# WangYuTum/odometry

Measured on AMD Instinct MI355X. Metric: tracked frames/sec (1241x376, 4-level pyramid), higher is better.
Workload: dtype f32

## Files before the change

### odometry_amd/csrc/kernels.hip.h

```cpp
#pragma once
#include <hip/hip_runtime.h>
#include "odo_math.h"

#ifndef ODO_PHASE_STAMPS
#define ODO_PHASE_STAMPS 0
#endif
#if ODO_PHASE_STAMPS
#define ODO_DBG(a) ((a).dbg)
#else
#define ODO_DBG(a) ((unsigned long long*)nullptr)
#endif

#ifndef ODO_KERNEL
#define ODO_KERNEL __global__
#define ODO_KERNEL_T __global__
#endif
#ifdef ODO_LM_CHAIN_TU
#define ODO_DEVICE_VAR static __device__
#else
#define ODO_DEVICE_VAR __device__
#endif

namespace odo {

// ... 1154 lines not shown
    if (lv) {
      while (!h.active && h.status == 0 && !h.finished) {
        const int next = (h.level < 0) ? n_levels - 1 : h.level - 1;
        if (next < stop_level) { h.finished = 1; break; }
        h.stop_reason = 0;
        h.level = next;
        h.iter = 0;
        h.err_last = 1e+10f;
        h.lambda = lambda0;
        h.inc = h.cur;
        h.max_iters = lv[next].max_iters;
        h.active = (h.status == 0 && h.max_iters > 0) ? 1 : 0;
#pragma unroll
        for (int c = 0; c < 4; c++) {
#pragma unroll
          for (int r = 0; r < 3; r++) Tn[c * 4 + r] = h.Tc[c * 3 + r];
          Tn[c * 4 + 3] = (c == 3) ? 1.0f : 0.0f;
        }
        new_T = true;
      }
      if (h.status != 0) h.finished = 1;
    }
    if (t == 0) {
      if (new_T) {
#pragma unroll
        for (int i = 0; i < 16; i++) s_sh.T[i] = Tn[i];
      }
      s_sh.level = h.level; s_sh.active = h.active; s_sh.status = h.status; s_sh.finished = h.finished;
    }
  }
  __syncthreads();
}

constexpr int kUpdThreads = 1024;
#define ODO_STAMP(i) do { if (STAMP && threadIdx.x == 0) stamps[i] = __builtin_readcyclecounter(); } while (0)
template <bool STAMP>
__device__ __forceinline__ void lm_update_body(LmState* __restrict__ st, const double* __restrict__ partials,
                                               int nblk, int expect_level, float precision, int max_iters,
                                               LmTraceRow* __restrict__ trace, float* __restrict__ cost_stat,
                                               int* __restrict__ host_prog, int seq,
                                               unsigned long long* __restrict__ stamps) {
  ODO_STAMP(0);
  if (!(st->active != 0 && st->level == expect_level)) {
    if (host_prog && threadIdx.x == 0) __hip_atomic_store(host_prog, seq, __ATOMIC_RELAXED, __HIP_MEMORY_SCOPE_SYSTEM);
    return;
  }
  __shared__ double sh[32][32];
  __shared__ double acc_sh[32];
  __shared__ LmState s_sh;
  const int t = threadIdx.x;
  const int q = t & 31, seg = t >> 5;
  double v = 0.0;
  if (q < ODO_NACC) {
    double v0 = 0.0, v1 = 0.0, v2 = 0.0, v3 = 0.0;
    int b = seg;
    for (; b + 96 < nblk; b += 128) {
      v0 += partials[(size_t)b * ODO_NACC + q];
      v1 += partials[(size_t)(b + 32) * ODO_NACC + q];
      v2 += partials[(size_t)(b + 64) * ODO_NACC + q];
      v3 += partials[(size_t)(b + 96) * ODO_NACC + q];
    }
    for (; b < nblk; b += 32) v0 += partials[(size_t)b * ODO_NACC + q];
    v = (v0 + v1) + (v2 + v3);
  }
  ODO_STAMP(1);
  sh[seg][q] = v;
// ... 232 lines not shown
  for (int rd = 0; rd < kCoarseRounds; rd++) my_cnt[rd] = __popcll(__ballot(rd < nr && valid[rd]));
  float sigma = 5.0f;
  int n_total = 0;
  for (int pass = 0; pass < kTdistMaxPasses; pass++) {
#pragma unroll
    for (int rd = 0; rd < kCoarseRounds; rd++) {
      const double ws = wave_sum64((rd < nr && valid[rd]) ? (double)tdist_term(e2[rd], sigma * sigma) : 0.0);
      if (lane == 0) { part[pass & 1][rd * kW + wv] = ws; if (pass == 0) cnt[rd * kW + wv] = my_cnt[rd]; }
    }
    __syncthreads();
    if (pass == 0) {
      int tot = 0;
#pragma unroll
      for (int i = 0; i < kCoarseChunks; i++) tot += cnt[i];
      n_total = tot;
    }
    double G = 0.0;
    if (lane < kCoarseChunks / 4) {
      const double* pv = &part[pass & 1][(lane >> 1) * kW + 4 * (lane & 1)];
      G = ((pv[0] + pv[1]) + pv[2]) + pv[3];
    }
    const double total = wave_sum64(G);
    const float nxt = (n_total > 0) ? tdist_next_sigma(total, n_total) : sigma;
    const bool done = (n_total == 0) || tdist_converged(nxt, sigma);
    sigma = nxt;
    if (done) break;
  }
  return sigma;
}
#if ODO_PHASE_STAMPS
ODO_DEVICE_VAR unsigned long long g_lm_diag[24];
#endif
constexpr unsigned long long kArmWaitTicks = 200000000ull;
template <bool kFull, bool kArmed = false>
__device__ __forceinline__ void lm_coarse_body(const StepArgs& a, const StepLaunch& q, int min_level, const unsigned* __restrict__ lv_src) {
#if ODO_PHASE_STAMPS
  const unsigned long long w_entry = (unsigned long long)wall_clock64();
#endif
  if (!kArmed && lm_chain_skip(a)) return;
  __builtin_amdgcn_s_setprio(3);
  lm_span_begin(q.span);
  __shared__ LmState s_sh;
  extern __shared__ __attribute__((aligned(16))) double red_sh[];
  __shared__ double acc_sh[32];
  __shared__ StepLevel lv_sh[ODO_MAX_LEVELS_K];
  __shared__ unsigned long long sm_sh[4];
  unsigned long long arm_g0 = 0;
  if (kArmed && threadIdx.x < 17) arm_g0 = __hip_atomic_load(a.arm + threadIdx.x, __ATOMIC_RELAXED, __HIP_MEMORY_SCOPE_SYSTEM);
  lm_copy_levels(lv_sh, lv_src);
  if (threadIdx.x == 0) {
#pragma unroll
    for (int i = 0; i < 4; i++) sm_sh[i] = 0;
  }
  __shared__ __attribute__((aligned(16))) float arm_pose_sh[16];
  __shared__ __attribute__((aligned(16))) int arm_verdict_sh4[4];
  if (kArmed) {
    if (threadIdx.x < 64) {
      const int lane = (int)threadIdx.x;
      unsigned long long g = arm_g0;
      bool got = __all(lane >= 17 || (int)(g >> 32) == a.token);
      const unsigned long long t0 = (unsigned long long)wall_clock64();
      for (int spin = 0; !got; spin++) {
        if (lane < 17) g = __hip_atomic_load(a.arm + lane, __ATOMIC_RELAXED, __HIP_MEMORY_SCOPE_SYSTEM);
        got = __all(lane >= 17 || (int)(g >> 32) == a.token);
        if (!got && (spin & 15) == 15 && (unsigned long long)wall_clock64() - t0 > (a.fine_wait ? (unsigned long long)a.fine_wait : kArmWaitTicks)) break;
      }
      if (lane < 16) arm_pose_sh[lane] = __uint_as_float((unsigned)g);
      if (lane == 16) arm_verdict_sh4[0] = got ? (int)(unsigned)g : 3;
    }
    __syncthreads();
    if (arm_verdict_sh4[0] == 3) {
      if (threadIdx.x < 64) {
        if (threadIdx.x < (int)(sizeof(LmState) / sizeof(int))) ((int*)&s_sh)[threadIdx.x] = 0;
        if (threadIdx.x == 0) { s_sh.status = -2; s_sh.active = 0; s_sh.finished = 1; }
      }
      __syncthreads();
      lm_fused_publish(s_sh, q.st_out, a.host_prog, q.seq, a.token, a.cost_stat, a.out, a.done_flag, a.final_state);
      return;
    }
    if (arm_verdict_sh4[0] != 1) return;
  } else {
    __syncthreads();
  }
#if ODO_PHASE_STAMPS
  const unsigned long long w_p1 = (unsigned long long)wall_clock64();
#endif
  lm_fused_prologue(q.st_in, q.part_in, lv_sh, a.n_levels, a.lambda0, a.precision, s_sh, red_sh, acc_sh, (kFull ? a.trace : (LmTraceRow*)nullptr), a.cost_stat, true,
                    kArmed ? arm_pose_sh : (q.first_of_solve ? a.init : nullptr), a.stop_level, (!kArmed && a.chain_in_token) ? a.chain_pose : nullptr);
#if ODO_PHASE_STAMPS
  const unsigned long long w_p2 = (unsigned long long)wall_clock64();
#endif
  LmHot hot;
  lm_hot_load(hot, s_sh);
  if (ODO_DBG(a) && threadIdx.x == 0 && q.seq < 56) ODO_DBG(a)[16 + 2 * q.seq] = wall_clock64();
  unsigned long long c_eval = 0, c_red = 0, c_sm = 0, c_it = 0, c_last = ODO_DBG(a) ? __builtin_readcyclecounter() : 0;
  const unsigned long long c_begin = c_last, w_begin = ODO_DBG(a) ? (unsigned long long)wall_clock64() : 0;
  auto lap = [&](unsigned long long& sum) {
    if (ODO_DBG(a)) { const unsigned long long now = __builtin_readcyclecounter(); sum += now - c_last; c_last = now; }
  };
  static_assert(kCoarseBlock == 2 * kLmBlock, "two 256-point virtual blocks per round");
  constexpr int kS = 8;
  constexpr int kVbMax = (kCoarseMaxPoints + kLmBlock - 1) / kLmBlock;
  __shared__ double part_sh[kVbMax][32];
  __shared__ double sc_part[2][kCoarseChunks];
  __shared__ int sc_cnt[kCoarseChunks];
  const int tl = threadIdx.x & (kLmBlock - 1), half = threadIdx.x >> 8;
  float* rows_sh = (float*)red_sh + half * (kRowFloats * RowBuf<kLmBlock>::W);
  const int my_q = tl / kS, my_s = tl % kS;
  int rowA = 0, rowB = 0;
  if (my_q < ODO_NACC) rows_of_quantity(my_q, &rowA, &rowB);
  PointK cpt[kCoarseRounds];
  bool cpt_ok[kCoarseRounds] = {false, false};
  int cpt_level = -1;
  for (int guard = 0; guard < 4096; guard++) {
    const bool run = (s_sh.active != 0 && s_sh.status == 0 && s_sh.level >= min_level);
    if (!run) break;
    c_it++;
    const StepLevel& L = lv_sh[s_sh.level];
    const float* I2u = lm_uniform_ptr(L.I2);
    float T[16];
#pragma unroll
    for (int i = 0; i < 16; i++) T[i] = s_sh.T[i];
    const int nvb = L.nblk;
    if (s_sh.level != cpt_level) {
      cpt_level = s_sh.level;
#pragma unroll
      for (int rd = 0; rd < kCoarseRounds; rd++) {
        const int vb = 2 * rd + half, idx = vb * kLmBlock + tl;
        cpt_ok[rd] = vb < nvb && idx < L.n;
        if (cpt_ok[rd]) cpt[rd] = load_point(L.pl, idx);
      }
    }
    float td_r[kCoarseRounds] = {0.0f, 0.0f}, td_J[kCoarseRounds][6] = {{0.0f, 0.0f, 0.0f, 0.0f, 0.0f, 0.0f}, {0.0f, 0.0f, 0.0f, 0.0f, 0.0f, 0.0f}};
    bool td_valid[kCoarseRounds] = {false, false};
    float td_scale_sqr = 1.0f;
    if ((kFull && a.robust == 2)) {
      float e2[kCoarseRounds];
#pragma unroll
      for (int rd = 0; rd < kCoarseRounds; rd++) {
        if (cpt_ok[rd]) td_valid[rd] = point_residual_g<kFull>(cpt[rd], T, L.k, I2u, L.rows, L.cols, &td_r[rd], td_J[rd]);
        e2[rd] = td_r[rd] * td_r[rd];
      }
      const float sg = coarse_tdist_sigma(sc_part, sc_cnt, e2, td_valid, (nvb + 1) / 2);
      td_scale_sqr = sg * sg;
    }
#pragma unroll
    for (int vb0 = 0; vb0 < 2 * kCoarseRounds; vb0 += 2) {
      if (vb0 >= nvb) break;
      const int vb = vb0 + half;
      float r = 0.0f, w = 0.0f, J[6] = {0.0f, 0.0f, 0.0f, 0.0f, 0.0f, 0.0f};
      bool valid = false;
      if ((kFull && a.robust == 2)) {
        r = td_r[vb0 / 2]; valid = td_valid[vb0 / 2];
#pragma unroll
        for (int i = 0; i < 6; i++) J[i] = td_J[vb0 / 2][i];
// ... 8 lines not shown
      rows_store_z(rows_sh, RowBuf<kLmBlock>::W, tl, J, w, r, valid);
      __syncthreads();
      if (vb0 == 0) lap(c_eval);
      double accq = 0.0;
      if (vb < nvb) {
        if (my_q < ODO_NACC) accq = rows_accumulate<kLmBlock, kS>(rows_sh, rowA, rowB, my_s, accq);
        accq = rows_butterfly8(accq);
      }
      if (nvb == 1) {
        if (half == 0 && my_q < ODO_NACC && my_s == 0) {
          double v = 0.0;
          v += accq;
          double acc = 0.0;
          acc += v;
#pragma unroll
          for (int g = 1; g < 8; g++) acc += 0.0;
          acc_sh[my_q] = acc;
        }
      } else if (vb < nvb && my_q < ODO_NACC && my_s == 0) {
        part_sh[vb][my_q] = accq;
      }
    }
    __syncthreads();
    if (nvb > 1) {
      const int fq = threadIdx.x & 31, fseg = threadIdx.x >> 5;
      double* fold_sh = red_sh;
      if (fseg < 8) {
        double v = 0.0;
        if (fq < ODO_NACC)
          for (int b = fseg; b < nvb; b += 8) v += part_sh[b][fq];
        fold_sh[fseg * 32 + fq] = v;
      }
      __syncthreads();
      if (threadIdx.x < ODO_NACC) {
        double acc = 0.0;
#pragma unroll
        for (int g = 0; g < 8; g++) acc += fold_sh[g * 32 + threadIdx.x];
        acc_sh[threadIdx.x] = acc;
      }
    }
    lap(c_red);
    lm_state_machine_hot(hot, lv_sh, a.n_levels, a.lambda0, a.precision, s_sh, acc_sh, (kFull ? a.trace : (LmTraceRow*)nullptr), a.cost_stat, true,
                         ODO_DBG(a) ? sm_sh : nullptr, a.stop_level);
    lap(c_sm);
  }
#if ODO_PHASE_STAMPS
  const unsigned long long w_loop_end = (unsigned long long)wall_clock64();
#endif
  if (threadIdx.x == 0) lm_hot_store(hot, s_sh);
  lm_fused_publish(s_sh, q.st_out, a.host_prog, q.seq, a.token, a.cost_stat, a.out, a.done_flag, a.final_state, chain_out_of(a));
#if ODO_PHASE_STAMPS
  if (ODO_DBG(a) && threadIdx.x == 0) {
    const unsigned long long now = (unsigned long long)wall_clock64();
    g_lm_diag[4] += w_begin - w_entry; g_lm_diag[5] += w_loop_end - w_begin; g_lm_diag[6] += now - w_loop_end;
    g_lm_diag[16] += w_p1 - w_entry; g_lm_diag[17] += w_p2 - w_p1; g_lm_diag[18] += w_begin - w_p2;
    if (g_lm_diag[1] && w_entry > g_lm_diag[1] && w_entry - g_lm_diag[1] < 100000ull) { g_lm_diag[7] += w_entry - g_lm_diag[1]; g_lm_diag[3] += w_entry - g_lm_diag[2]; g_lm_diag[14] += 1; }
    g_lm_diag[0] = now; g_lm_diag[8] += 1;
  }
#endif
  if (ODO_DBG(a) && threadIdx.x == 0) {
    if (q.seq < 56) ODO_DBG(a)[16 + 2 * q.seq + 1] = wall_clock64();
    ODO_DBG(a)[0] += c_eval; ODO_DBG(a)[1] += c_red; ODO_DBG(a)[2] += c_sm; ODO_DBG(a)[3] += c_it;
    ODO_DBG(a)[4] += __builtin_readcyclecounter() - c_begin; ODO_DBG(a)[5] += 1;
    ODO_DBG(a)[6] += (unsigned long long)wall_clock64() - w_begin;
#pragma unroll
    for (int i = 0; i < 4; i++) ODO_DBG(a)[8 + i] += sm_sh[i];
  }
  lm_span_end(q.span);
}

#ifdef ODO_LM_CHAIN_TU
static __global__ void __launch_bounds__(kCoarseBlock) lm_coarse_kernel(StepArgs a, int min_level) {
  const StepLaunch q = {a.st_in, a.st_out, a.part_in, a.part_out, a.seq, a.first_of_solve, a.span};
  lm_coarse_body<false>(a, q, min_level, lm_kernarg_words());
}
static __global__ void __launch_bounds__(kCoarseBlock) lm_coarse_armed_kernel(StepArgs a, int min_level) {
  const StepLaunch q = {a.st_in, a.st_out, a.part_in, a.part_out, a.seq, a.first_of_solve, a.span};
  lm_coarse_body<false, true>(a, q, min_level, lm_kernarg_words());
}
static __global__ void __launch_bounds__(kCoarseBlock) lm_coarse_full_kernel(StepArgs a, int min_level) {
  const StepLaunch q = {a.st_in, a.st_out, a.part_in, a.part_out, a.seq, a.first_of_solve, a.span};
  lm_coarse_body<true>(a, q, min_level, lm_kernarg_words());
}
#endif
template <bool kFull>
__device__ __forceinline__ void lm_coarse_batch_entry(const StepArgs* __restrict__ table, int seq, int first_of_solve, unsigned long long* span) {
  const StepArgs& a = table[blockIdx.y];
  const StepLaunch q = {a.st2[seq & 1], a.st2[(seq + 1) & 1], a.part2[seq & 1], a.part2[(seq + 1) & 1], seq, first_of_solve, span};
  lm_coarse_body<kFull>(a, q, a.min_level, (const unsigned*)&table[blockIdx.y]);
}
ODO_KERNEL void __launch_bounds__(kCoarseBlock) lm_coarse_kernel_batch(const StepArgs* __restrict__ table, int seq, int first_of_solve,
                                                                       unsigned long long* span) {
  lm_coarse_batch_entry<false>(table, seq, first_of_solve, span);
}
ODO_KERNEL void __launch_bounds__(kCoarseBlock) lm_coarse_full_kernel_batch(const StepArgs* __restrict__ table, int seq, int first_of_solve,
                                                                            unsigned long long* span) {
  lm_coarse_batch_entry<true>(table, seq, first_of_solve, span);
}

constexpr int kFineGran = 2 * ODO_NACC;
constexpr int kFineRowsMax = 160;
constexpr int kFineChunk = 8;
constexpr unsigned kFineWaitTicks = 400000u;
struct FineDeadline {
  unsigned long long t0, c0;
  unsigned limit;
  static __device__ __forceinline__ FineDeadline begin(unsigned limit_ticks) {
    return FineDeadline{(unsigned long long)wall_clock64(), (unsigned long long)__builtin_readcyclecounter(), limit_ticks};
  }
  __device__ __forceinline__ bool expired(int spin) const {
    if ((spin & 31) != 31) return false;
// ... 157 lines not shown
    }
    FineG2 g = {0, 0, 0, 0};
    unsigned long long gc = 0;
    bool all = false;
    FineDeadline dl = {0ull, 0ull, wait_limit};
    __builtin_amdgcn_s_setprio(0);
    for (int spin = 0; !all; spin++) {
      if (spin == 1) dl = FineDeadline::begin(wait_limit);
      if (spin > 0) { if (dl.expired(spin)) break; __builtin_amdgcn_s_sleep(1); }
      bool mine = true;
      if (lane < nvb) {
        g = *(const volatile FineG2Global*)(sums + 2 * lane);
        if (pass == 0) gc = __hip_atomic_load(cnts + lane, __ATOMIC_RELAXED, __HIP_MEMORY_SCOPE_AGENT);
        mine = (g.x == tag) && (g.z == tag) && (pass != 0 || (unsigned)gc == tag);
      }
      all = __all(mine);
    }
    __builtin_amdgcn_s_setprio(3);
    if (!all) { if (lane == 0) *bail = 1; break; }
    double part = 0.0, cnt = 0.0;
    if (lane < nvb) {
      part = __longlong_as_double((long long)(((unsigned long long)g.y << 32) | (unsigned long long)g.w));
      if (pass == 0) cnt = (double)(unsigned)(gc >> 32);
    }
    const double total = wave_sum64(part);
    if (pass == 0) n_total = (int)wave_sum64(cnt);
    const float nxt = (n_total > 0) ? tdist_next_sigma(total, n_total) : sigma;
    const bool done = (n_total == 0) || tdist_converged(nxt, sigma);
    sigma = nxt;
    if (done) break;
  }
  return sigma;
}
template <bool kTdist, bool kTrace>
__device__ __forceinline__ void lm_fine_body(const StepArgs& a, const StepLaunch& q, int K, int w, unsigned long long* __restrict__ xbuf,
                                             int fault, int lo_level, const unsigned* __restrict__ lv_src) {
#if ODO_PHASE_STAMPS
  const unsigned long long w_entry = (unsigned long long)wall_clock64();
#endif
  __builtin_amdgcn_s_setprio(3);
  const int t = threadIdx.x, tl = t & (kLmBlock - 1), half = t >> 8;
  const bool publisher = (w == 0);
  if (publisher && t == 0 && q.span) atomicMin(q.span, (unsigned long long)wall_clock64());
  __shared__ LmState s_sh;
  __shared__ double fold_sh[8 * 32];
  __shared__ double acc_sh[32];
  __shared__ StepLevel lv_sh[ODO_MAX_LEVELS_K];
  __shared__ float rows_sh2[2][kRowFloats * RowBuf<kLmBlock>::W];
  __shared__ int bail_sh, local_sh;
  __shared__ unsigned long long sm_sh[4];
  float* rows_sh = rows_sh2[half];
  const unsigned tag_base = a.fine_epoch << 8;
  unsigned long long* place = xbuf + 2 * kFineRowsMax * kFineGran;
  const unsigned wait_limit = a.fine_wait ? a.fine_wait : kFineWaitTicks;
  lm_copy_levels(lv_sh, lv_src);
  if (t == 0) {
    bail_sh = 0;
    local_sh = 0;
#pragma unroll
    for (int i = 0; i < 4; i++) sm_sh[i] = 0;
    __hip_atomic_store(place + w, ((unsigned long long)(unsigned)fine_xcc_id() << 32) | tag_base, __ATOMIC_RELAXED, __HIP_MEMORY_SCOPE_AGENT);
  }
  __syncthreads();
  lm_fused_prologue(q.st_in, q.part_in, lv_sh, a.n_levels, a.lambda0, a.precision, s_sh, fold_sh, acc_sh, (kTrace ? a.trace : (LmTraceRow*)nullptr), a.cost_stat,
                    publisher, q.first_of_solve ? a.init : nullptr, a.stop_level, a.chain_in_token ? a.chain_pose : nullptr);
  LmHot hot;
  lm_hot_load(hot, s_sh);
  if (t < 64) {
    bool same = true, got = false;
    if (t < K) {
      unsigned long long pw = 0;
      const FineDeadline dl = FineDeadline::begin(wait_limit);
      for (int spin = 0; !got; spin++) {
        pw = __hip_atomic_load(place + t, __ATOMIC_RELAXED, __HIP_MEMORY_SCOPE_AGENT);
        got = ((unsigned)pw == tag_base);
        if (!got && dl.expired(spin)) break;
      }
      same = got && ((int)(pw >> 32) == fine_xcc_id());
    } else {
      got = true;
    }
    const bool all_got = __all(got), all_same = __all(same);
    if (t == 0) { local_sh = (all_got && all_same) ? 1 : 0; if (!all_got) bail_sh = 1; }
  }
  __syncthreads();
  const bool local = local_sh != 0;
  constexpr int kS = 8;
  const int my_q = tl / kS, my_s = tl % kS;
  int rowA = 0, rowB = 0;
  if (my_q < ODO_NACC) rows_of_quantity(my_q, &rowA, &rowB);
  const int fq = t & 31, fseg = t >> 5;
  PointK pt;
  bool pt_ok = false;
  int pt_level = -1;
  unsigned long long c_eval = 0, c_xchg = 0, c_sm = 0, c_it = 0, c_last = ODO_DBG(a) ? __builtin_readcyclecounter() : 0;
#if ODO_PHASE_STAMPS
  unsigned long long c_first = 0, n_first = 0;
#endif
  const unsigned long long c_begin = c_last, w_begin = ODO_DBG(a) ? (unsigned long long)wall_clock64() : 0;
  auto lap = [&](unsigned long long& sum) {
    if (ODO_DBG(a)) { const unsigned long long now = __builtin_readcyclecounter(); sum += now - c_last; c_last = now; }
  };
  for (int ev = 0; ev < 4096; ev++) {
    const bool run = (s_sh.active != 0 && s_sh.status == 0 && !s_sh.finished && !bail_sh && s_sh.level >= lo_level);
    if (!run) break;
    c_it++;
    const StepLevel& L = lv_sh[s_sh.level];
    const float* I2u = lm_uniform_ptr(L.I2);
    const int nblk = L.nblk;
    const unsigned tag = tag_base + 1u + (unsigned)(ev % 255);
    unsigned long long* buf = xbuf + (size_t)(ev & 1) * kFineRowsMax * kFineGran;
    float T[16];
#pragma unroll
    for (int i = 0; i < 16; i++) T[i] = s_sh.T[i];
#if ODO_PHASE_STAMPS
    const bool first_of_level = (s_sh.level != pt_level);
#endif
    const bool resident = (nblk <= 2 * K) && (L.n <= nblk * kLmBlock);
    if (resident) {
      const int vb = w + half * K;
      if (s_sh.level != pt_level) {
        pt_level = s_sh.level;
        const int idx = vb * kLmBlock + tl;
        pt_ok = vb < nblk && idx < L.n;
        if (pt_ok) pt = load_point(L.pl, idx);
      }
      float r = 0.0f, wgt = 0.0f, J[6] = {0.0f, 0.0f, 0.0f, 0.0f, 0.0f, 0.0f};
      bool valid = false;
      if (pt_ok && point_residual_g<kTdist || kTrace>(pt, T, L.k, I2u, L.rows, L.cols, &r, J)) {
        wgt = robust_weight(r, (kTdist || kTrace) ? a.robust : (a.robust == 1 ? 1 : 0), a.huber_delta, 1.0f);
        valid = true;
      }
      if (kTdist && w < nblk) {
        __shared__ double td_ws_sh[2][8];
        __shared__ int td_cnt_sh[8];
        const float sg = fine_tdist_sigma(xbuf + kFineScaleOff, vb * 4 + (tl >> 6), 4 * nblk,
                                          ((a.fine_epoch & 0xfffu) << 20) | (((unsigned)ev & 0x3ffu) << 10), r * r, valid, local, wait_limit, &bail_sh,
                                          td_ws_sh, td_cnt_sh);
        if (valid) wgt = robust_weight(r, 2, a.huber_delta, sg * sg);
      }
      rows_store_z(rows_sh, RowBuf<kLmBlock>::W, tl, J, wgt, r, valid);
      __syncthreads();
      if (bail_sh) break;
      if (vb < nblk) {
        double accq = 0.0;
        if (my_q < ODO_NACC) accq = rows_accumulate<kLmBlock, kS>(rows_sh, rowA, rowB, my_s, accq);
        accq = rows_butterfly8(accq);
// ... 32 lines not shown
    double v = 0.0;
    __builtin_amdgcn_s_setprio(0);
    if (fq < ODO_NACC && fseg < 8) {
      for (int b0 = fseg; b0 < nblk; b0 += 8 * kFineChunk) {
        FineG2 g2[kFineChunk];
        bool all = false;
        FineDeadline dl = {0ull, 0ull, wait_limit};
        for (int spin = 0; !all; spin++) {
          if (spin == 1) dl = FineDeadline::begin(wait_limit);
          if (spin > 0) { if (dl.expired(spin)) break; __builtin_amdgcn_s_sleep(1); }
          all = true;
#pragma unroll
          for (int u = 0; u < kFineChunk; u++) {
            const int b = b0 + 8 * u;
            if (b < nblk) g2[u] = *(const volatile FineG2Global*)(buf + (size_t)b * kFineGran + 2 * fq);
          }
#pragma unroll
          for (int u = 0; u < kFineChunk; u++) {
            const int b = b0 + 8 * u;
            if (b < nblk) all = all && (g2[u].x == tag) && (g2[u].z == tag);
          }
        }
        if (!all) bail_sh = 1;
#pragma unroll
        for (int u = 0; u < kFineChunk; u++) {
          const int b = b0 + 8 * u;
          if (b < nblk) v += __longlong_as_double((long long)(((unsigned long long)g2[u].y << 32) | (unsigned long long)g2[u].w));
        }
      }
    }
    __builtin_amdgcn_s_setprio(3);
    if (fseg < 8) fold_sh[fseg * 32 + fq] = v;
    __syncthreads();
    if (t < ODO_NACC) {
      double acc = 0.0;
#pragma unroll
      for (int g = 0; g < 8; g++) acc += fold_sh[g * 32 + t];
      acc_sh[t] = acc;
    }
    lap(c_xchg);
    if (bail_sh) break;
    lm_state_machine_hot(hot, lv_sh, a.n_levels, a.lambda0, a.precision, s_sh, acc_sh, (kTrace ? a.trace : (LmTraceRow*)nullptr), a.cost_stat, publisher,
                         (ODO_DBG(a) && publisher) ? sm_sh : nullptr, a.stop_level);
    lap(c_sm);
  }
#if ODO_PHASE_STAMPS
  const unsigned long long w_loop_end = (unsigned long long)wall_clock64();
#endif
  if (t == 0) lm_hot_store(hot, s_sh);
  if (bail_sh && t == 0) { s_sh.status = -2; s_sh.active = 0; s_sh.finished = 1; }
  __syncthreads();
  if (publisher) {
    lm_fused_publish(s_sh, q.st_out, a.host_prog, q.seq, a.token, a.cost_stat, a.out, a.done_flag, a.final_state, chain_out_of(a));
#if ODO_PHASE_STAMPS
    const unsigned long long w_published = (unsigned long long)wall_clock64();
#endif
    if (ODO_DBG(a) && t == 0) { ODO_DBG(a)[128] += c_eval; ODO_DBG(a)[129] += c_xchg; ODO_DBG(a)[130] += c_sm; ODO_DBG(a)[131] += c_it; ODO_DBG(a)[132] += 1; ODO_DBG(a)[133] += local ? 1 : 0;
      ODO_DBG(a)[134] += __builtin_readcyclecounter() - c_begin; ODO_DBG(a)[135] += (unsigned long long)wall_clock64() - w_begin;
#pragma unroll
      for (int i = 0; i < 4; i++) ODO_DBG(a)[136 + i] += sm_sh[i]; }
    if (t == 0 && q.span) atomicMax(q.span + 1, (unsigned long long)wall_clock64());
#if ODO_PHASE_STAMPS
    if (ODO_DBG(a) && t == 0) {
      const unsigned long long now = w_published;
      g_lm_diag[2] = w_loop_end;
      g_lm_diag[19] += c_first; g_lm_diag[20] += n_first;
      g_lm_diag[9] += w_begin - w_entry; g_lm_diag[10] += w_loop_end - w_begin; g_lm_diag[11] += now - w_loop_end;
      if (g_lm_diag[0] && w_entry > g_lm_diag[0] && w_entry - g_lm_diag[0] < 100000ull) { g_lm_diag[12] += w_entry - g_lm_diag[0]; g_lm_diag[15] += 1; }
      g_lm_diag[1] = now; g_lm_diag[13] += 1;
    }
#endif
  }
}
ODO_DEVICE_VAR unsigned g_lm_fine_dispatch[2];
__device__ __forceinline__ bool lm_fine_mid_dispatch() {
  return __hip_atomic_load(&g_lm_fine_dispatch[0], __ATOMIC_RELAXED, __HIP_MEMORY_SCOPE_AGENT) !=
         __hip_atomic_load(&g_lm_fine_dispatch[1], __ATOMIC_RELAXED, __HIP_MEMORY_SCOPE_AGENT);
}
template <bool kTdist, bool kTrace>
__device__ __forceinline__ void lm_fine_entry(const StepArgs& a, int K, unsigned long long* __restrict__ xbuf, int fault, int lo_level,
                                              unsigned* dispatch_words) {
  if (threadIdx.x == 0) {
    if (blockIdx.x == 0) __hip_atomic_store(&dispatch_words[0], a.fine_dispatch, __ATOMIC_RELAXED, __HIP_MEMORY_SCOPE_AGENT);
    if (blockIdx.x == gridDim.x - 1) __hip_atomic_store(&dispatch_words[1], a.fine_dispatch, __ATOMIC_RELAXED, __HIP_MEMORY_SCOPE_AGENT);
  }
  if (!fine_on_home(a.fine_home) || lm_chain_skip(a)) return;
  const StepLaunch q = {a.st_in, a.st_out, a.part_in, a.part_out, a.seq, a.first_of_solve, a.span};
  lm_fine_body<kTdist, kTrace>(a, q, K, (int)(blockIdx.x >> 3), xbuf, fault, lo_level, lm_kernarg_words());
}
#ifdef ODO_LM_CHAIN_TU
static __global__ void __launch_bounds__(kFineThreads) lm_fine_kernel(StepArgs a, int K, unsigned long long* __restrict__ xbuf, int fault,
                                                               int lo_level, unsigned* dispatch_words) {
  lm_fine_entry<false, false>(a, K, xbuf, fault, lo_level, dispatch_words);
}
static __global__ void __launch_bounds__(kFineThreads) lm_fine_trace_kernel(StepArgs a, int K, unsigned long long* __restrict__ xbuf, int fault,
                                                                     int lo_level, unsigned* dispatch_words) {
  lm_fine_entry<false, true>(a, K, xbuf, fault, lo_level, dispatch_words);
}
static __global__ void __launch_bounds__(kFineThreads) lm_fine_tdist_kernel(StepArgs a, int K, unsigned long long* __restrict__ xbuf, int fault,
                                                                     int lo_level, unsigned* dispatch_words) {
  lm_fine_entry<true, true>(a, K, xbuf, fault, lo_level, dispatch_words);
}
#endif
template <bool kTrace>
__device__ __forceinline__ void lm_fine_batch_entry(const StepArgs* __restrict__ table, int n, int K, int seq, int first_of_solve,
                                                    unsigned long long* span, int fault, const XccIds& xcc, unsigned* dispatch_words) {
  int r = (int)(blockIdx.x & 7u);
  if (xcc.id[0] >= 0) {
    const int mine = fine_xcc_id();
#pragma unroll
    for (int c = 0; c < 8; c++) if (xcc.id[c] == mine) r = c;
  }
  if (threadIdx.x == 0 && n > 0) {
    if (blockIdx.x == 0) __hip_atomic_store(&dispatch_words[0], table[0].fine_dispatch, __ATOMIC_RELAXED, __HIP_MEMORY_SCOPE_AGENT);
    if (blockIdx.x == gridDim.x - 1) __hip_atomic_store(&dispatch_words[1], table[0].fine_dispatch, __ATOMIC_RELAXED, __HIP_MEMORY_SCOPE_AGENT);
  }
  const int wa = (int)(blockIdx.x >> 3);
  const int i = (wa / K) * 8 + r, w = wa % K;
  if (i >= n) return;
  const StepArgs& a = table[i];
  const StepLaunch q = {a.st2[seq & 1], a.st2[(seq + 1) & 1], a.part2[seq & 1], a.part2[(seq + 1) & 1], seq, first_of_solve,
                        (i == 0) ? span : nullptr};
  if (a.fine_lo >= a.min_level) {
    if (w == 0) lm_fine_body<false, kTrace>(a, q, 1, 0, a.xbuf, 0, ODO_MAX_LEVELS_K + 1, (const unsigned*)&table[i]);
    return;
  }
// ... 822 lines not shown
```

### odometry_amd/csrc/odo_math.h

```cpp
#pragma once
#include <math.h>
#include <stdint.h>

#if defined(__HIPCC__)
#define ODO_HD __host__ __device__ __forceinline__
#else
#define ODO_HD static inline
#endif

#define ODO_NACC 29

namespace odo {

struct LevelK {
  double fl;
  float cx, cy;
  int bilinear;
};

ODO_HD float cx_level(float c, int level) {
  float v = c;
  for (int i = 0; i < level; i++) v = (v + 0.5f) / 2.0f + 0.5f;
  return v;
}
// ... 410 lines not shown
  s->active = (s->status == 0 && max_iters > 0) ? 1 : 0;
  s->max_iters = max_iters;
  se3_to_colmajor(s->inc, s->T);
}

ODO_HD bool lm_decide(LmState* s, const double acc[ODO_NACC], float precision) {
  s->n_evals++;
  {
    const int li = s->level & 7;
#pragma unroll
    for (int i = 0; i < 8; i++) s->iters_level[i] += (i == li) ? 1 : 0;
  }
  if (!(acc[28] > 0.0)) {
    s->status = -1;
    s->active = 0;
    return false;
  }
  const float err_now = (float)(acc[27] / acc[28]);
  s->err_now = err_now;
  if (err_now > s->err_last) {
    s->lambda = s->lambda * 5.0f;
    if (s->lambda > 1e+5f) { s->active = 0; s->stop_reason = 2; return false; }
    s->cur = s->last;
  } else {
    s->cur = s->inc;
    s->last = s->cur;
    const float err_diff = err_now / s->err_last;
    if (err_diff > precision) { s->active = 0; s->stop_reason = 1; return false; }
    s->err_last = err_now;
    s->lambda = fmaxf(s->lambda / 5.0f, 1e-5f);
  }
  return true;
}
ODO_HD void lm_apply_step(LmState* s, int max_iters) {
  Se3 d;
  se3_exp(s->delta, &d);
  se3_left_update(d, s->cur, &s->inc);
  se3_to_colmajor(s->inc, s->T);
  s->iter++;
  if (!(max_iters > s->iter)) { s->active = 0; s->stop_reason = 3; }
}
ODO_HD void lm_consume(LmState* s, const double acc[ODO_NACC], float precision, int max_iters) {
  if (!lm_decide(s, acc, precision)) return;
  solve_damped(acc, s->lambda, s->delta);
  lm_apply_step(s, max_iters);
}

ODO_HD void motion_angles3(const float* T, float ang[3]) {
  Se3 s;
  se3_from_colmajor(T, &s);
  float R[9];
  quat_to_rot(s, R);
  ang[0] = atan2f(R[7] - R[5], R[4] + R[8]);
  ang[1] = atan2f(R[2] - R[6], R[0] + R[8]);
  ang[2] = atan2f(R[3] - R[1], R[0] + R[4]);
}
ODO_HD float motion_magnitude(const float* T, const float w[6]) {
  float ang[3];
  motion_angles3(T, ang);
  const float mot[6] = {fabsf(ang[0]), fabsf(ang[1]), fabsf(ang[2]), fabsf(T[12]), fabsf(T[13]), fabsf(T[14])};
  float mag = 0.0f;
  for (int i = 0; i < 6; i++) mag += mot[i] * w[i];
  return mag;
}

ODO_HD float atan2_approx(float y, float x) {
// ... 55 lines not shown
```

Measured before the change: 4063.

## Speculatively solve both LM accept/reject steps in parallel waves during state machine

Adds a roles-based LM state machine in which wave 0 evaluates the accept/reject decision while waves 1 and 2 each solve the damped system for one of the two possible lambda outcomes and build the resulting pose in LDS. The next iteration then picks the precomputed pose by a selector instead of running the solve serially after the decision. This is meant to take the 6x6 solve and SE3 exponential off the serial critical path of each coarse and fine LM iteration. The cost is duplicated solve work, extra LDS state, and extra carry bookkeeping. It is enabled by default for the coarse and fine kernels, but not for the trace variants. Span timing is also moved in the armed path.

```diff
diff --git a/odometry_amd/csrc/kernels.hip.h b/odometry_amd/csrc/kernels.hip.h
--- a/odometry_amd/csrc/kernels.hip.h
+++ b/odometry_amd/csrc/kernels.hip.h
@@ -1210,6 +1210,182 @@
   __syncthreads();
 }
 
+#ifndef ODO_LM_ROLES
+#define ODO_LM_ROLES 3
+#endif
+struct LmRolesLds {
+  float T[2][3][16];
+  float inc[2][2][8];
+  float d[2][2][8];
+  float Tc[2][16];
+  double acc[2][32];
+  float lambda[2];
+  int sel;
+};
+struct LmRolesCarry {
+  const float* Tp;
+  int par;
+  int pend_step;
+  int pend_inc;
+};
+__device__ __forceinline__ void lm_roles_begin(LmRolesCarry& rc, const LmHot& h, LmRolesLds& R) {
+  rc.Tp = nullptr; rc.par = 0; rc.pend_step = -1; rc.pend_inc = 0;
+  if (threadIdx.x == 0) {
+    R.lambda[0] = h.lambda;
+#pragma unroll
+    for (int c = 0; c < 4; c++) {
+#pragma unroll
+      for (int r = 0; r < 3; r++) { R.Tc[0][c * 4 + r] = h.Tc[c * 3 + r]; }
+      R.Tc[0][c * 4 + 3] = (c == 3) ? 1.0f : 0.0f;
+      R.Tc[1][c * 4 + 3] = (c == 3) ? 1.0f : 0.0f;
+    }
+  }
+}
+__device__ __forceinline__ void lm_roles_load_T(LmRolesCarry& rc, const LmState& s_sh, const LmRolesLds& R, float T[16]) {
+  const int sel = R.sel;
+  rc.Tp = sel ? &R.T[0][0][0] + (sel - 1) * 16 : s_sh.T;
+#pragma unroll
+  for (int i = 0; i < 16; i++) T[i] = rc.Tp[i];
+}
+__device__ __forceinline__ void lm_roles_settle(LmRolesCarry& rc, LmHot& h, LmState& s_sh, const LmRolesLds& R) {
+  if (rc.pend_step >= 0) {
+    const float* pi = R.inc[rc.par ^ 1][rc.pend_step];
+    const float* pd = R.d[rc.par ^ 1][rc.pend_step];
+    if (rc.pend_inc) { h.inc.qw = pi[0]; h.inc.qx = pi[1]; h.inc.qy = pi[2]; h.inc.qz = pi[3]; h.inc.tx = pi[4]; h.inc.ty = pi[5]; h.inc.tz = pi[6]; }
+    if ((threadIdx.x & 63) == 0) {
+#pragma unroll
+      for (int i = 0; i < 6; i++) s_sh.delta[i] = pd[i];
+    }
+    rc.pend_step = -1;
+  }
+}
+__device__ __forceinline__ void lm_roles_finish(LmRolesCarry& rc, LmHot& h, LmState& s_sh, const LmRolesLds& R) {
+  lm_roles_settle(rc, h, s_sh, R);
+  const int sel = R.sel;
+  if (sel && (threadIdx.x & 63) == 0) {
+    const float* p = &R.T[0][0][0] + (sel - 1) * 16;
+#pragma unroll
+    for (int i = 0; i < 16; i++) s_sh.T[i] = p[i];
+  }
+}
+__device__ __forceinline__ void lm_state_machine_roles(LmHot& h, LmRolesCarry& rc, LmRolesLds& R, const StepLevel* lv, int n_levels,
+                                                       float lambda0, float precision, LmState& s_sh, const double* acc_sh,
+                                                       const double* fold_sh, bool from_fold, unsigned long long* smdbg = nullptr,
+                                                       int stop_level = 0) {
+  const int wave = __builtin_amdgcn_readfirstlane((int)(threadIdx.x >> 6));
+  const int lane = (int)(threadIdx.x & 63);
+  const int par = rc.par;
+  if (wave == 0) {
+    unsigned long long c0 = smdbg ? __builtin_readcyclecounter() : 0;
+    lm_roles_settle(rc, h, s_sh, R);
+    const int lvl0 = h.level;
+    float Tprev[12];
+#pragma unroll
+    for (int c = 0; c < 4; c++)
+#pragma unroll
+      for (int r = 0; r < 3; r++) Tprev[c * 3 + r] = rc.Tp[c * 4 + r];
+    double s27 = 0.0, s28 = 0.0;
+    if (from_fold) {
+#pragma unroll
+      for (int g = 0; g < 8; g++) { s27 += fold_sh[g * 32 + 27]; s28 += fold_sh[g * 32 + 28]; }
+    } else {
+      s27 = acc_sh[27]; s28 = acc_sh[28];
+    }
+    h.n_evals++;
+    if (lane == 0) s_sh.iters_level[lvl0 & 7] += 1;
+    const LmOutcome o = lm_outcome(s27, s28, h.err_last, h.lambda, h.iter, h.max_iters, precision, h.active, h.status, h.stop_reason);
+    h.lambda = o.lambda; h.err_last = o.err_last; h.iter = o.iter; h.active = o.active; h.status = o.status; h.stop_reason = o.stop_reason;
+    if (o.accepted) {
+      h.cur = h.inc;
+#pragma unroll
+      for (int i = 0; i < 12; i++) h.Tc[i] = Tprev[i];
+    }
+    int sel = -1;
+    if (o.step) { sel = 1 + 3 * par + (o.step - 1); rc.pend_step = o.step - 1; rc.pend_inc = 1; }
+    if (smdbg && lane == 0) { smdbg[0] += __builtin_readcyclecounter() - c0; smdbg[3] += 1; }
+    if (lane == 0 && o.have_err) s_sh.err_now = o.err_now;
+    if (lv) {
+      while (!h.active && h.status == 0 && !h.finished) {
+        const int next = (h.level < 0) ? n_levels - 1 : h.level - 1;
+        if (next < stop_level) { h.finished = 1; break; }
+        h.stop_reason = 0;
+        h.level = next;
+        h.iter = 0;
+        h.err_last = 1e+10f;
+        h.lambda = lambda0;
+        h.inc = h.cur;
+        rc.pend_inc = 0;
+        h.max_iters = lv[next].max_iters;
+        h.active = (h.status == 0 && h.max_iters > 0) ? 1 : 0;
+        sel = 1 + 3 * par + 2;
+      }
+      if (h.status != 0) h.finished = 1;
+    }
+    if (lane == 0) {
+      if (sel == 1 + 3 * par + 2) {
+#pragma unroll
+        for (int c = 0; c < 4; c++) {
+#pragma unroll
+          for (int r = 0; r < 3; r++) R.T[par][2][c * 4 + r] = h.Tc[c * 3 + r];
+          R.T[par][2][c * 4 + 3] = (c == 3) ? 1.0f : 0.0f;
+        }
+      }
+      if (sel >= 0) R.sel = sel;
+      s_sh.level = h.level; s_sh.active = h.active; s_sh.status = h.status; s_sh.finished = h.finished;
+      R.lambda[par ^ 1] = h.lambda;
+#pragma unroll
+      for (int c = 0; c < 4; c++)
+#pragma unroll
+        for (int r = 0; r < 3; r++) R.Tc[par ^ 1][c * 4 + r] = h.Tc[c * 3 + r];
+    }
+  } else if (wave <= 2) {
+    unsigned long long c1 = smdbg ? __builtin_readcyclecounter() : 0, c2 = c1;
+    const int k = wave - 1;
+    const float lam = R.lambda[par];
+    const float* Cp = k ? R.Tc[par] : rc.Tp;
+    float C[16];
+#pragma unroll
+    for (int c = 0; c < 4; c++) {
+#pragma unroll
+      for (int r = 0; r < 3; r++) C[c * 4 + r] = Cp[c * 4 + r];
+      C[c * 4 + 3] = (c == 3) ? 1.0f : 0.0f;
+    }
+    const double* accp = acc_sh;
+    if (from_fold) {
+      if (lane < ODO_NACC) {
+        double acc = 0.0;
+#pragma unroll
+        for (int g = 0; g < 8; g++) acc += fold_sh[g * 32 + lane];
+        R.acc[k][lane] = acc;
+      }
+      accp = R.acc[k];
+    }
+    const float lam_k = k ? lam * 5.0f : fmaxf(lam / 5.0f, 1e-5f);
+    float d[6];
+    solve_damped_wave_regs(accp, lam_k, d);
+    if (smdbg) { asm volatile("" ::"v"(d[0]), "v"(d[5])); c2 = __builtin_readcyclecounter(); }
+    Se3 dd, inc;
+    se3_exp_wave(d, &dd);
+    se3_left_update_mat(dd, C, &inc);
+    float Tn[16];
+    se3_to_colmajor(inc, Tn);
+    if (lane == 0) {
+      float* pi = R.inc[par][k];
+      pi[0] = inc.qw; pi[1] = inc.qx; pi[2] = inc.qy; pi[3] = inc.qz; pi[4] = inc.tx; pi[5] = inc.ty; pi[6] = inc.tz;
+#pragma unroll
+      for (int i = 0; i < 6; i++) R.d[par][k][i] = d[i];
+#pragma unroll
+      for (int i = 0; i < 16; i++) R.T[par][k][i] = Tn[i];
+    }
+    if (smdbg && k == 0 && lane == 0) {
+      asm volatile("" ::"v"(Tn[0]), "v"(Tn[14]));
+      smdbg[1] += c2 - c1; smdbg[2] += __builtin_readcyclecounter() - c2;
+    }
+  }
+  rc.par = par ^ 1;
+  __syncthreads();
+}
+
 constexpr int kUpdThreads = 1024;
 #define ODO_STAMP(i) do { if (STAMP && threadIdx.x == 0) stamps[i] = __builtin_readcyclecounter(); } while (0)
 template <bool STAMP>
@@ -1508,25 +1684,27 @@
 ODO_DEVICE_VAR unsigned long long g_lm_diag[24];
 #endif
 constexpr unsigned long long kArmWaitTicks = 200000000ull;
-template <bool kFull, bool kArmed = false>
+template <bool kFull, bool kArmed = false, bool kRoles = false>
 __device__ __forceinline__ void lm_coarse_body(const StepArgs& a, const StepLaunch& q, int min_level, const unsigned* __restrict__ lv_src) {
 #if ODO_PHASE_STAMPS
   const unsigned long long w_entry = (unsigned long long)wall_clock64();
 #endif
   if (!kArmed && lm_chain_skip(a)) return;
   __builtin_amdgcn_s_setprio(3);
-  lm_span_begin(q.span);
+  if (!kArmed) lm_span_begin(q.span);
   __shared__ LmState s_sh;
   extern __shared__ __attribute__((aligned(16))) double red_sh[];
   __shared__ double acc_sh[32];
   __shared__ StepLevel lv_sh[ODO_MAX_LEVELS_K];
   __shared__ unsigned long long sm_sh[4];
+  __shared__ LmRolesLds roles_sh;
   unsigned long long arm_g0 = 0;
   if (kArmed && threadIdx.x < 17) arm_g0 = __hip_atomic_load(a.arm + threadIdx.x, __ATOMIC_RELAXED, __HIP_MEMORY_SCOPE_SYSTEM);
   lm_copy_levels(lv_sh, lv_src);
   if (threadIdx.x == 0) {
 #pragma unroll
     for (int i = 0; i < 4; i++) sm_sh[i] = 0;
+    if (kRoles) roles_sh.sel = 0;
   }
   __shared__ __attribute__((aligned(16))) float arm_pose_sh[16];
   __shared__ __attribute__((aligned(16))) int arm_verdict_sh4[4];
@@ -1551,10 +1729,13 @@
         if (threadIdx.x == 0) { s_sh.status = -2; s_sh.active = 0; s_sh.finished = 1; }
       }
       __syncthreads();
+      lm_span_begin(q.span);
       lm_fused_publish(s_sh, q.st_out, a.host_prog, q.seq, a.token, a.cost_stat, a.out, a.done_flag, a.final_state);
+      lm_span_end(q.span);
       return;
     }
-    if (arm_verdict_sh4[0] != 1) return;
+    lm_span_begin(q.span);
+    if (arm_verdict_sh4[0] != 1) { lm_span_end(q.span); return; }
   } else {
     __syncthreads();
   }
@@ -1568,6 +1749,8 @@
 #endif
   LmHot hot;
   lm_hot_load(hot, s_sh);
+  LmRolesCarry rc;
+  if (kRoles) lm_roles_begin(rc, hot, roles_sh);
   if (ODO_DBG(a) && threadIdx.x == 0 && q.seq < 56) ODO_DBG(a)[16 + 2 * q.seq] = wall_clock64();
   unsigned long long c_eval = 0, c_red = 0, c_sm = 0, c_it = 0, c_last = ODO_DBG(a) ? __builtin_readcyclecounter() : 0;
   const unsigned long long c_begin = c_last, w_begin = ODO_DBG(a) ? (unsigned long long)wall_clock64() : 0;
@@ -1595,8 +1778,12 @@
     const StepLevel& L = lv_sh[s_sh.level];
     const float* I2u = lm_uniform_ptr(L.I2);
     float T[16];
-#pragma unroll
-    for (int i = 0; i < 16; i++) T[i] = s_sh.T[i];
+    if (kRoles) {
+      lm_roles_load_T(rc, s_sh, roles_sh, T);
+    } else {
+#pragma unroll
+      for (int i = 0; i < 16; i++) T[i] = s_sh.T[i];
+    }
     const int nvb = L.nblk;
     if (s_sh.level != cpt_level) {
       cpt_level = s_sh.level;
@@ -1671,7 +1858,7 @@
         fold_sh[fseg * 32 + fq] = v;
       }
       __syncthreads();
-      if (threadIdx.x < ODO_NACC) {
+      if (!kRoles && threadIdx.x < ODO_NACC) {
         double acc = 0.0;
 #pragma unroll
         for (int g = 0; g < 8; g++) acc += fold_sh[g * 32 + threadIdx.x];
@@ -1679,13 +1866,18 @@
       }
     }
     lap(c_red);
-    lm_state_machine_hot(hot, lv_sh, a.n_levels, a.lambda0, a.precision, s_sh, acc_sh, (kFull ? a.trace : (LmTraceRow*)nullptr), a.cost_stat, true,
-                         ODO_DBG(a) ? sm_sh : nullptr, a.stop_level);
+    if (kRoles)
+      lm_state_machine_roles(hot, rc, roles_sh, lv_sh, a.n_levels, a.lambda0, a.precision, s_sh, acc_sh, red_sh, nvb > 1,
+                             ODO_DBG(a) ? sm_sh : nullptr, a.stop_level);
+    else
+      lm_state_machine_hot(hot, lv_sh, a.n_levels, a.lambda0, a.precision, s_sh, acc_sh, (kFull ? a.trace : (LmTraceRow*)nullptr), a.cost_stat, true,
+                           ODO_DBG(a) ? sm_sh : nullptr, a.stop_level);
     lap(c_sm);
   }
 #if ODO_PHASE_STAMPS
   const unsigned long long w_loop_end = (unsigned long long)wall_clock64();
 #endif
+  if (kRoles && threadIdx.x < 64) lm_roles_finish(rc, hot, s_sh, roles_sh);
   if (threadIdx.x == 0) lm_hot_store(hot, s_sh);
   lm_fused_publish(s_sh, q.st_out, a.host_prog, q.seq, a.token, a.cost_stat, a.out, a.done_flag, a.final_state, chain_out_of(a));
 #if ODO_PHASE_STAMPS
@@ -1711,11 +1903,11 @@
 #ifdef ODO_LM_CHAIN_TU
 static __global__ void __launch_bounds__(kCoarseBlock) lm_coarse_kernel(StepArgs a, int min_level) {
   const StepLaunch q = {a.st_in, a.st_out, a.part_in, a.part_out, a.seq, a.first_of_solve, a.span};
-  lm_coarse_body<false>(a, q, min_level, lm_kernarg_words());
+  lm_coarse_body<false, false, (ODO_LM_ROLES & 1) != 0>(a, q, min_level, lm_kernarg_words());
 }
 static __global__ void __launch_bounds__(kCoarseBlock) lm_coarse_armed_kernel(StepArgs a, int min_level) {
   const StepLaunch q = {a.st_in, a.st_out, a.part_in, a.part_out, a.seq, a.first_of_solve, a.span};
-  lm_coarse_body<false, true>(a, q, min_level, lm_kernarg_words());
+  lm_coarse_body<false, true, (ODO_LM_ROLES & 1) != 0>(a, q, min_level, lm_kernarg_words());
 }
 static __global__ void __launch_bounds__(kCoarseBlock) lm_coarse_full_kernel(StepArgs a, int min_level) {
   const StepLaunch q = {a.st_in, a.st_out, a.part_in, a.part_out, a.seq, a.first_of_solve, a.span};
@@ -1939,7 +2131,7 @@
   }
   return sigma;
 }
-template <bool kTdist, bool kTrace>
+template <bool kTdist, bool kTrace, bool kRoles = false>
 __device__ __forceinline__ void lm_fine_body(const StepArgs& a, const StepLaunch& q, int K, int w, unsigned long long* __restrict__ xbuf,
                                              int fault, int lo_level, const unsigned* __restrict__ lv_src) {
 #if ODO_PHASE_STAMPS
@@ -1956,6 +2148,7 @@
   __shared__ float rows_sh2[2][kRowFloats * RowBuf<kLmBlock>::W];
   __shared__ int bail_sh, local_sh;
   __shared__ unsigned long long sm_sh[4];
+  __shared__ LmRolesLds roles_sh;
   float* rows_sh = rows_sh2[half];
   const unsigned tag_base = a.fine_epoch << 8;
   unsigned long long* place = xbuf + 2 * kFineRowsMax * kFineGran;
@@ -1964,6 +2157,7 @@
   if (t == 0) {
     bail_sh = 0;
     local_sh = 0;
+    if (kRoles) roles_sh.sel = 0;
 #pragma unroll
     for (int i = 0; i < 4; i++) sm_sh[i] = 0;
     __hip_atomic_store(place + w, ((unsigned long long)(unsigned)fine_xcc_id() << 32) | tag_base, __ATOMIC_RELAXED, __HIP_MEMORY_SCOPE_AGENT);
@@ -1973,6 +2167,8 @@
                     publisher, q.first_of_solve ? a.init : nullptr, a.stop_level, a.chain_in_token ? a.chain_pose : nullptr);
   LmHot hot;
   lm_hot_load(hot, s_sh);
+  LmRolesCarry rc;
+  if (kRoles) lm_roles_begin(rc, hot, roles_sh);
   if (t < 64) {
     bool same = true, got = false;
     if (t < K) {
@@ -2018,8 +2214,12 @@
     const unsigned tag = tag_base + 1u + (unsigned)(ev % 255);
     unsigned long long* buf = xbuf + (size_t)(ev & 1) * kFineRowsMax * kFineGran;
     float T[16];
-#pragma unroll
-    for (int i = 0; i < 16; i++) T[i] = s_sh.T[i];
+    if (kRoles) {
+      lm_roles_load_T(rc, s_sh, roles_sh, T);
+    } else {
+#pragma unroll
+      for (int i = 0; i < 16; i++) T[i] = s_sh.T[i];
+    }
 #if ODO_PHASE_STAMPS
     const bool first_of_level = (s_sh.level != pt_level);
 #endif
@@ -2118,7 +2318,7 @@
     __builtin_amdgcn_s_setprio(3);
     if (fseg < 8) fold_sh[fseg * 32 + fq] = v;
     __syncthreads();
-    if (t < ODO_NACC) {
+    if (!kRoles && t < ODO_NACC) {
       double acc = 0.0;
 #pragma unroll
       for (int g = 0; g < 8; g++) acc += fold_sh[g * 32 + t];
@@ -2126,13 +2326,18 @@
     }
     lap(c_xchg);
     if (bail_sh) break;
-    lm_state_machine_hot(hot, lv_sh, a.n_levels, a.lambda0, a.precision, s_sh, acc_sh, (kTrace ? a.trace : (LmTraceRow*)nullptr), a.cost_stat, publisher,
-                         (ODO_DBG(a) && publisher) ? sm_sh : nullptr, a.stop_level);
+    if (kRoles)
+      lm_state_machine_roles(hot, rc, roles_sh, lv_sh, a.n_levels, a.lambda0, a.precision, s_sh, acc_sh, fold_sh, true,
+                             (ODO_DBG(a) && publisher) ? sm_sh : nullptr, a.stop_level);
+    else
+      lm_state_machine_hot(hot, lv_sh, a.n_levels, a.lambda0, a.precision, s_sh, acc_sh, (kTrace ? a.trace : (LmTraceRow*)nullptr), a.cost_stat, publisher,
+                           (ODO_DBG(a) && publisher) ? sm_sh : nullptr, a.stop_level);
     lap(c_sm);
   }
 #if ODO_PHASE_STAMPS
   const unsigned long long w_loop_end = (unsigned long long)wall_clock64();
 #endif
+  if (kRoles && t < 64) lm_roles_finish(rc, hot, s_sh, roles_sh);
   if (t == 0) lm_hot_store(hot, s_sh);
   if (bail_sh && t == 0) { s_sh.status = -2; s_sh.active = 0; s_sh.finished = 1; }
   __syncthreads();
@@ -2163,7 +2368,7 @@
   return __hip_atomic_load(&g_lm_fine_dispatch[0], __ATOMIC_RELAXED, __HIP_MEMORY_SCOPE_AGENT) !=
          __hip_atomic_load(&g_lm_fine_dispatch[1], __ATOMIC_RELAXED, __HIP_MEMORY_SCOPE_AGENT);
 }
-template <bool kTdist, bool kTrace>
+template <bool kTdist, bool kTrace, bool kRoles = false>
 __device__ __forceinline__ void lm_fine_entry(const StepArgs& a, int K, unsigned long long* __restrict__ xbuf, int fault, int lo_level,
                                               unsigned* dispatch_words) {
   if (threadIdx.x == 0) {
@@ -2172,12 +2377,12 @@
   }
   if (!fine_on_home(a.fine_home) || lm_chain_skip(a)) return;
   const StepLaunch q = {a.st_in, a.st_out, a.part_in, a.part_out, a.seq, a.first_of_solve, a.span};
-  lm_fine_body<kTdist, kTrace>(a, q, K, (int)(blockIdx.x >> 3), xbuf, fault, lo_level, lm_kernarg_words());
+  lm_fine_body<kTdist, kTrace, kRoles>(a, q, K, (int)(blockIdx.x >> 3), xbuf, fault, lo_level, lm_kernarg_words());
 }
 #ifdef ODO_LM_CHAIN_TU
 static __global__ void __launch_bounds__(kFineThreads) lm_fine_kernel(StepArgs a, int K, unsigned long long* __restrict__ xbuf, int fault,
                                                                int lo_level, unsigned* dispatch_words) {
-  lm_fine_entry<false, false>(a, K, xbuf, fault, lo_level, dispatch_words);
+  lm_fine_entry<false, false, (ODO_LM_ROLES & 2) != 0>(a, K, xbuf, fault, lo_level, dispatch_words);
 }
 static __global__ void __launch_bounds__(kFineThreads) lm_fine_trace_kernel(StepArgs a, int K, unsigned long long* __restrict__ xbuf, int fault,
                                                                      int lo_level, unsigned* dispatch_words) {
diff --git a/odometry_amd/csrc/odo_math.h b/odometry_amd/csrc/odo_math.h
--- a/odometry_amd/csrc/odo_math.h
+++ b/odometry_amd/csrc/odo_math.h
@@ -466,6 +466,43 @@
   }
   return true;
 }
+struct LmOutcome {
+  int step;
+  int accepted;
+  int have_err;
+  float err_now;
+  float lambda, err_last;
+  int iter, active, status, stop_reason;
+};
+ODO_HD LmOutcome lm_outcome(double sum_err, double sum_n, float err_last, float lambda, int iter, int max_iters, float precision,
+                            int active, int status, int stop_reason) {
+  LmOutcome o;
+  o.step = 0; o.accepted = 0; o.have_err = 0; o.err_now = 0.0f;
+  o.lambda = lambda; o.err_last = err_last; o.iter = iter; o.active = active; o.status = status; o.stop_reason = stop_reason;
+  if (!(sum_n > 0.0)) {
+    o.status = -1;
+    o.active = 0;
+    return o;
+  }
+  const float err_now = (float)(sum_err / sum_n);
+  o.err_now = err_now;
+  o.have_err = 1;
+  if (err_now > err_last) {
+    o.lambda = lambda * 5.0f;
+    if (o.lambda > 1e+5f) { o.active = 0; o.stop_reason = 2; return o; }
+    o.step = 2;
+  } else {
+    o.accepted = 1;
+    const float err_diff = err_now / err_last;
+    if (err_diff > precision) { o.active = 0; o.stop_reason = 1; return o; }
+    o.err_last = err_now;
+    o.lambda = fmaxf(lambda / 5.0f, 1e-5f);
+    o.step = 1;
+  }
+  o.iter = iter + 1;
+  if (!(max_iters > o.iter)) { o.active = 0; o.stop_reason = 3; }
+  return o;
+}
 ODO_HD void lm_apply_step(LmState* s, int max_iters) {
   Se3 d;
   se3_exp(s->delta, &d);
```

New measurement: 4108 (median of 2 runs). About the same (+1.1%).
